# Lu-Zhan/Pano-NeRF

Hardware: AMD Instinct MI355X
Metric: rays/sec (train step) (higher is better)
Workload: dtype f32 (2xfp16 split products, fp32 accumulate; weight-gradient operands h_l / delta_l / r_l / hdot_l stored with 16 significant bits, 'Q24')

## Files before the change

pano-nerf_amd/csrc/pn_wgrad.hip:

```cpp
#include "pn_chain.h"

#ifdef PN_TRACE_WG
__device__ unsigned long long g_chain_trace[64];
extern "C" int pn_chain_trace_read(unsigned long long* out) {
    return hipMemcpyFromSymbol(out, HIP_SYMBOL(g_chain_trace), sizeof(unsigned long long) * 64) == hipSuccess ? 0 : -4;
}
#endif

struct WSeg {
    const float* X;
    const float* Y;
    int64_t nhalf;
    int FX, FY;
    int bias;
    const uint32_t* ax;
    const uint32_t* ay;
};
struct WgArgs {
    WSeg seg[4];
    int nseg;
    int64_t half_total, per;
    float* slab;
    int64_t slab_stride;
    int bias;
};
constexpr int WG_MAXJ = 8;
struct WgMulti {
    WgArgs job[WG_MAXJ];
};

template <int NP>
__device__ __forceinline__ f32x16 mfma_split32(const BFrag<NP>& a, const BFrag<NP>& b, f32x16 v) {
    if constexpr (NP == 3) {
        v = __builtin_amdgcn_mfma_f32_32x32x16_bf16(a.p[2], b.p[0], v, 0, 0, 0);
        v = __builtin_amdgcn_mfma_f32_32x32x16_bf16(a.p[0], b.p[2], v, 0, 0, 0);
        v = __builtin_amdgcn_mfma_f32_32x32x16_bf16(a.p[1], b.p[1], v, 0, 0, 0);
        v = __builtin_amdgcn_mfma_f32_32x32x16_bf16(a.p[1], b.p[0], v, 0, 0, 0);
        v = __builtin_amdgcn_mfma_f32_32x32x16_bf16(a.p[0], b.p[1], v, 0, 0, 0);
        v = __builtin_amdgcn_mfma_f32_32x32x16_bf16(a.p[0], b.p[0], v, 0, 0, 0);
    } else if constexpr (NP == 2) {
        v = __builtin_amdgcn_mfma_f32_32x32x16_f16(a.p[1], b.p[0], v, 0, 0, 0);
        v = __builtin_amdgcn_mfma_f32_32x32x16_f16(a.p[0], b.p[1], v, 0, 0, 0);
        v = __builtin_amdgcn_mfma_f32_32x32x16_f16(a.p[0], b.p[0], v, 0, 0, 0);
    } else {
        v = __builtin_amdgcn_mfma_f32_32x32x16_bf16(a.p[0], b.p[0], v, 0, 0, 0);
    }
    return v;
}
#define WG_LD(p) __builtin_nontemporal_load(p)
template <int NP, int TM, int TN, int WM, int WN, bool X24 = false, bool Y24 = false>
__global__ __launch_bounds__(64 * WM * WN) void k_chain_wgrad(WgMulti multi) {
    const WgArgs& a = multi.job[blockIdx.y];
    static_assert(!(X24 || Y24) || NP == 2, "Q24 tensors exist with fp16 pairs only");
    static_assert(!X24 || Y24, "combinations in use: (0,0), (0,1), (1,1)");
    constexpr bool ROT = X24 || Y24;
    constexpr int NTH = 64 * WM * WN, TMW = 32 * TM * WM, TNW = 32 * TN * WN;
    constexpr int PX = TMW * 16, PY = TNW * 16;
    constexpr int BUF = NP * (PX + PY);
    typedef typename TEl<NP>::type TE;
    constexpr int PPR = 16 * (int)sizeof(TE) / 16;
    constexpr int SPP = 16 / PPR;
    constexpr int CX = X24 ? 0 : TMW * PPR, CY = Y24 ? 0 : TNW * PPR;
    constexpr int LX = X24 ? 1 : (CX + NTH - 1) / NTH, LY = Y24 ? 1 : (CY + NTH - 1) / NTH;
    constexpr int UX = X24 ? TMW : 0, UY = Y24 ? TNW : 0;
    constexpr int LU = (UX + UY + NTH - 1) / NTH;
    static_assert(UX % 64 == 0, "a wave's units are all X or all Y");
    __shared__ __attribute__((aligned(16))) unsigned short smem[2 * BUF];
    const int tid = threadIdx.x, lane = tid & 63;
    const int wid = __builtin_amdgcn_readfirstlane(tid >> 6);
    const int wm = wid / WN, wn = wid % WN;
    const int64_t h0 = (int64_t)blockIdx.x * a.per;
    if (h0 >= a.half_total) return;
    int64_t h1 = h0 + a.per;
    if (h1 > a.half_total) h1 = a.half_total;

    f32x16 acc[TM][TN];
#pragma unroll
    for (int i = 0; i < TM; ++i)
#pragma unroll
        for (int j = 0; j < TN; ++j)
#pragma unroll
            for (int e = 0; e < 16; ++e) acc[i][j][e] = 0.f;
    float bsum[LX];
#pragma unroll
    for (int i = 0; i < LX; ++i) bsum[i] = 0.f;
    float bsum4[LU > 0 ? LU : 1][4] = {};

    constexpr int NSET = (X24 && LU == 1) ? 4 : ((NP <= 2 && (X24 ? 0 : LX) + (Y24 ? 0 : LY) + 3 * LU <= 4) ? 3 : 2);
    f32x4 xr[NSET][LX], yr[NSET][LY];
    f32x4 ur[NSET][LU > 0 ? LU : 1][3];
    constexpr bool ALT = (WM * WN == 8 && TM == 2 && TN == 4) && (X24 || Y24 || NP == 1);
    auto unit_of = [&](int i) { return tid + NTH * i; };
    float bw[NSET] = {};
    int sx[NSET] = {}, sy[NSET] = {}, unit = 0;
    auto seg_exps = [&](const WSeg& S, int& ex, int& ey) {
        ex = scale_exp(__uint_as_float(*S.ax), EXP_CAP_Z);
        ey = scale_exp(__uint_as_float(*S.ay), EXP_CAP_Z);
        int over = ex + ey - unit;
        const int rx = over < ex + 126 ? over : ex + 126;
        ex -= rx;
        ey -= over - rx;
        if (ey < -126) ey = -126;
    };
    if constexpr (NP == 2) {
        unit = 1 << 20;
        for (int i = 0; i < a.nseg; ++i) {
            const int e = scale_exp(__uint_as_float(*a.seg[i].ax), EXP_CAP_Z) + scale_exp(__uint_as_float(*a.seg[i].ay), EXP_CAP_Z);
            unit = e < unit ? e : unit;
        }
    }
    int csg = 0, cFX = a.seg[0].FX, cFY = a.seg[0].FY, csx = 0, csy = 0;
    int64_t cbase = 0, cend = a.seg[0].nhalf;
    const TE* cX = reinterpret_cast<const TE*>(a.seg[0].X);
    const TE* cY = reinterpret_cast<const TE*>(a.seg[0].Y);
    float cbw = a.seg[0].bias ? 1.f : 0.f;
    if constexpr (NP == 2) seg_exps(a.seg[0], csx, csy);
    auto load = [&](int64_t h, int set) __attribute__((always_inline)) {
        while (csg + 1 < a.nseg && h >= cend) {
            ++csg;
            const WSeg& S = a.seg[csg];
            cbase = cend;
            cend += S.nhalf;
            cX = reinterpret_cast<const TE*>(S.X);
            cY = reinterpret_cast<const TE*>(S.Y);
            cFX = S.FX;
            cFY = S.FY;
            cbw = S.bias ? 1.f : 0.f;
            if constexpr (NP == 2) seg_exps(S, csx, csy);
        }
        const int64_t hb = h - cbase;
        bw[set] = cbw;
        if constexpr (NP == 2) {
            sx[set] = csx;
            sy[set] = csy;
        }
        const int64_t blk = hb;
        const TE* xb = cX + blk * ((int64_t)cFX * TILE);
        const TE* yb = cY + blk * ((int64_t)cFY * TILE);
        if constexpr (!X24) {
#pragma unroll
            for (int i = 0; i < LX; ++i) {
                const int idx = tid + NTH * i;
                if (CX % NTH == 0 || idx < CX) xr[set][i] = WG_LD(reinterpret_cast<const f32x4*>(xb + (idx / PPR) * TILE + (idx % PPR) * SPP));
            }
        }
        if constexpr (!Y24) {
#pragma unroll
            for (int i = 0; i < LY; ++i) {
                const int idx = tid + NTH * i;
                if (CY % NTH == 0 || idx < CY) yr[set][i] = WG_LD(reinterpret_cast<const f32x4*>(yb + (idx / PPR) * TILE + (idx % PPR) * SPP));
            }
        }
        if constexpr (X24 || Y24) {
            const unsigned char* xq = reinterpret_cast<const unsigned char*>(cX) + blk * ((int64_t)cFX * 48);
            const unsigned char* yq = reinterpret_cast<const unsigned char*>(cY) + blk * ((int64_t)cFY * 48);
#pragma unroll
            for (int i = 0; i < LU; ++i) {
                const int u = unit_of(i);
                if ((UX + UY) % NTH == 0 || u < UX + UY) {
                    const f32x4* p = reinterpret_cast<const f32x4*>(u < UX ? xq + u * 48 : yq + (u - UX) * 48);
                    ur[set][i][0] = p[0];
                    ur[set][i][1] = p[1];
                    ur[set][i][2] = p[2];
                }
            }
        }
    };
    auto put = [&](unsigned short* plane0, int pstride, int idx, const f32x4& v, int ex) {
        if constexpr (NP == 1) {
            const int f = idx >> 1, q = idx & 1;
            *reinterpret_cast<f32x4*>(plane0 + f * 16 + ((q ^ ((f >> 3) & 1)) << 3)) = v;
            return;
        }
        const int f0 = idx >> 2, q = idx & 3;
        const int f = ROT ? ((f0 & ~3) | ((f0 + (f0 >> 2)) & 3)) : f0;
        const int o = f * 16 + (((q >> 1) ^ ((f >> 3) & 1)) << 3) + (q & 1) * 4;
        if constexpr (NP == 2) {
            const float s = pow2f(ex);
            const float x4[4] = {v[0], v[1], v[2], v[3]};
            uint32_t h2[2], l2[2];
            split2_pairs<2>(x4, s, h2, l2);
            *reinterpret_cast<uint2*>(plane0 + o) = make_uint2(h2[0], h2[1]);
            *reinterpret_cast<uint2*>(plane0 + pstride + o) = make_uint2(l2[0], l2[1]);
        } else {
            typedef __bf16 bf16x4 __attribute__((ext_vector_type(4)));
            bf16x4 hv, mv, lv;
#pragma unroll
            for (int c = 0; c < 4; ++c) {
                const __bf16 hb = (__bf16)v[c];
                hv[c] = hb;
                if constexpr (NP == 3) {
                    const float r1 = v[c] - (float)hb;
                    const __bf16 mb = (__bf16)r1;
                    mv[c] = mb;
                    lv[c] = (__bf16)(r1 - (float)mb);
                }
            }
            *reinterpret_cast<bf16x4*>(plane0 + o) = hv;
            if constexpr (NP == 3) {
                *reinterpret_cast<bf16x4*>(plane0 + pstride + o) = mv;
                *reinterpret_cast<bf16x4*>(plane0 + 2 * pstride + o) = lv;
            }
        }
    };
    auto put_unit = [&](unsigned short* plane0, int pstride, int u, const f32x4 (&r)[3], int ex, float* bs, float w) {
        typedef uint32_t u32x4 __attribute__((ext_vector_type(4)));
        uint32_t d[12];
#pragma unroll
        for (int k = 0; k < 3; ++k) {
            const u32x4 t = __builtin_bit_cast(u32x4, r[k]);
#pragma unroll
            for (int c = 0; c < 4; ++c) d[4 * k + c] = t[c];
        }
        float e[4][4];
#pragma unroll
        for (int sm = 0; sm < 4; ++sm) {
            e[sm][0] = __uint_as_float(d[3 * sm] << 8);
            e[sm][1] = __uint_as_float(__builtin_amdgcn_perm(d[3 * sm + 1], d[3 * sm], 0x0504030cu));
            e[sm][2] = __uint_as_float(__builtin_amdgcn_perm(d[3 * sm + 2], d[3 * sm + 1], 0x0403020cu));
            e[sm][3] = __uint_as_float(d[3 * sm + 2] & 0xffffff00u);
        }
        const int qb = u >> 2, sg = u & 3;
#pragma unroll
        for (int f = 0; f < 4; ++f) {
            const f32x4 v{e[0][f], e[1][f], e[2][f], e[3][f]};
            put(plane0, pstride, (4 * qb + f) * 4 + sg, v, ex);
            if (bs) bs[f] += w * ((v[0] + v[1]) + (v[2] + v[3]));
        }
    };
    auto stage = [&](int buf, int set) __attribute__((always_inline)) {
        unsigned short* xs = smem + buf * BUF;
        unsigned short* ys = xs + NP * PX;
        if constexpr (PN_ABL_WG & 2) {
            if constexpr (X24 || Y24) {
#pragma unroll
                for (int i = 0; i < LU; ++i) asm volatile("" ::"v"(ur[set][i][0]), "v"(ur[set][i][1]), "v"(ur[set][i][2]));
            }
            if constexpr (!X24) {
#pragma unroll
                for (int i = 0; i < LX; ++i) asm volatile("" ::"v"(xr[set][i]));
            }
            if constexpr (!Y24) {
#pragma unroll
                for (int i = 0; i < LY; ++i) asm volatile("" ::"v"(yr[set][i]));
            }
            return;
        }
        if constexpr (X24 || Y24) {
#pragma unroll
            for (int i = 0; i < LU; ++i) {
                const int u = unit_of(i);
                if ((UX + UY) % NTH == 0 || u < UX + UY) {
                    if (u < UX) put_unit(xs, PX, u, ur[set][i], sx[set], bsum4[i], bw[set]);
                    else put_unit(ys, PY, u - UX, ur[set][i], sy[set], nullptr, 0.f);
                }
            }
        }
        if constexpr (!X24)
#pragma unroll
        for (int i = 0; i < LX; ++i) {
            const int idx = tid + NTH * i;
            if (CX % NTH == 0 || idx < CX) {
                put(xs, PX, idx, xr[set][i], sx[set]);
                if constexpr (NP == 1) {
                    const bf16x8 hv = __builtin_bit_cast(bf16x8, xr[set][i]);
                    float t = 0.f;
#pragma unroll
                    for (int c = 0; c < 8; ++c) t += (float)hv[c];
                    bsum[i] += bw[set] * t;
                } else {
                    bsum[i] += bw[set] * ((xr[set][i][0] + xr[set][i][1]) + (xr[set][i][2] + xr[set][i][3]));
                }
            }
        }
        if constexpr (!Y24)
#pragma unroll
        for (int i = 0; i < LY; ++i) {
            const int idx = tid + NTH * i;
            if (CY % NTH == 0 || idx < CY) put(ys, PY, idx, yr[set][i], sy[set]);
        }
    };
    const int fr = lane & 31, fh = lane >> 5;
    auto frag = [&](const unsigned short* plane, int feature) {
        if constexpr (ROT) feature = (feature & ~3) | ((feature + (feature >> 2)) & 3);
        return *reinterpret_cast<const typename PlaneOf<NP>::type*>(plane + feature * 16 + ((fh ^ ((feature >> 3) & 1)) << 3));
    };
    auto compute = [&](int buf) __attribute__((always_inline)) {
        if constexpr (PN_ABL_WG & 1) return;
        const unsigned short* xs = smem + buf * BUF;
        const unsigned short* ys = xs + NP * PX;
        if constexpr (X24) {
            BFrag<NP> af[TM];
#pragma unroll
            for (int i = 0; i < TM; ++i)
#pragma unroll
                for (int p = 0; p < NP; ++p) af[i].p[p] = frag(xs + p * PX, 32 * (wm * TM + i) + fr);
#pragma unroll
            for (int j = 0; j < TN; ++j) {
                BFrag<NP> bf;
#pragma unroll
                for (int p = 0; p < NP; ++p) bf.p[p] = frag(ys + p * PY, 32 * (wn * TN + j) + fr);
#pragma unroll
                for (int i = 0; i < TM; ++i) acc[i][j] = mfma_split32<NP>(af[i], bf, acc[i][j]);
            }
            return;
        }
        typedef typename PlaneOf<NP>::type Frag;
        auto lds_of = [](const unsigned short* q) { return (uint32_t)(uintptr_t)(lds_ptr_t)q; };
        auto fidx = [&](int feature) {
            if constexpr (ROT) feature = (feature & ~3) | ((feature + (feature >> 2)) & 3);
            return feature * 16 + ((fh ^ ((feature >> 3) & 1)) << 3);
        };
        const uint32_t xa = lds_of(xs) + 2 * fidx(32 * (wm * TM) + fr), ya = lds_of(ys) + 2 * fidx(32 * (wn * TN) + fr);
        auto rd = [](Frag& dst, uint32_t addr, auto off) {
            asm volatile("ds_read_b128 %0, %1 offset:%2" : "=v"(dst) : "v"(addr), "n"(decltype(off)::value) : "memory");
        };
        static_assert(2 * NP * PX + 1024 * TM < 65536 && 2 * NP * PY + 1024 * TN < 65536, "16-bit offset field of ds_read_b128");
        BFrag<NP> af[TM];
        BFrag<NP> bf[2];
        auto read_b = [&](auto jc, BFrag<NP>& f) {
            constexpr int J = decltype(jc)::value;
            static_for<NP>([&](auto pc) {
                constexpr int P = decltype(pc)::value;
                rd(f.p[P], ya, std::integral_constant<int, 1024 * J + 2 * P * PY>{});
            });
        };
        auto settle = [&](auto left, BFrag<NP>& f) {
            constexpr int L = decltype(left)::value;
#pragma unroll
            for (int p = 0; p < NP; ++p) {
                if (p == 0) asm volatile("s_waitcnt lgkmcnt(%1)" : "+v"(f.p[p]) : "n"(L) : "memory");
                else asm volatile("" : "+v"(f.p[p]));
            }
        };
        read_b(std::integral_constant<int, 0>{}, bf[0]);
        static_for<TM>([&](auto ic) {
            constexpr int I = decltype(ic)::value;
            static_for<NP>([&](auto pc) {
                constexpr int P = decltype(pc)::value;
                rd(af[I].p[P], xa, std::integral_constant<int, 1024 * I + 2 * P * PX>{});
            });
        });
        if constexpr (TN > 1) {
            read_b(std::integral_constant<int, 1>{}, bf[1]);
            settle(std::integral_constant<int, NP>{}, bf[0]);
        } else {
            settle(std::integral_constant<int, 0>{}, bf[0]);
        }
#pragma unroll
        for (int i = 0; i < TM; ++i)
#pragma unroll
            for (int p = 0; p < NP; ++p) asm volatile("" : "+v"(af[i].p[p]));
        static_for<TN>([&](auto jc) {
            constexpr int J = decltype(jc)::value;
#pragma unroll
            for (int i = 0; i < TM; ++i) acc[i][J] = mfma_split32<NP>(af[i], bf[J & 1], acc[i][J]);
            if constexpr (J + 2 < TN) {
                __builtin_amdgcn_sched_barrier(0);
                read_b(std::integral_constant<int, J + 2>{}, bf[J & 1]);
            }
            if constexpr (J + 1 < TN) {
                if constexpr (J + 2 < TN) settle(std::integral_constant<int, NP>{}, bf[(J + 1) & 1]);
                else settle(std::integral_constant<int, 0>{}, bf[(J + 1) & 1]);
            }
        });
    };
#ifdef PN_TRACE_WG
    unsigned long long tw[4] = {0, 0, 0, 0};
#define WGT(i, expr)                                                   \
    do {                                                               \
        const unsigned long long t0_ = __builtin_amdgcn_s_memtime();   \
        expr;                                                          \
        asm volatile("s_waitcnt lgkmcnt(0)" ::: "memory");             \
        tw[i] += __builtin_amdgcn_s_memtime() - t0_;                   \
    } while (0)
#else
#define WGT(i, expr) expr
#endif
    auto one = [&](auto kc, int64_t h) __attribute__((always_inline)) {
        constexpr int K = decltype(kc)::value;
        if (h + K < h1) {
            WGT(0, stage(K % 2, K % NSET));
            WGT(1, __syncthreads());
            WGT(2, if (h + K + NSET < h1) load(h + K + NSET, K % NSET));
            WGT(3, compute(K % 2));
        }
    };
    if constexpr (ALT) {
        const int t = wid >= (WM * WN) / 2 ? 1 : 0;
        const int64_t n = h1 - h0;
        auto clampd = [&](int64_t hb) { return h0 + (hb < n ? hb : n - 1); };
        if (n > 0) {
            load(h0, 0);
            stage(0, 0);
            load(clampd(1), 0);
            if (t && 1 < n) stage(1, 0);
#pragma unroll
            for (int sidx = 1; sidx < NSET; ++sidx) load(clampd(sidx + t), sidx);
            load(clampd(NSET + t), 0);
            __syncthreads();
            constexpr int TRIPA = NSET == 3 ? 6 : (NSET == 4 ? 4 : 2);
            auto alt = [&](auto kc, auto guard, int64_t k0) __attribute__((always_inline)) {
                constexpr int K = decltype(kc)::value;
                if (!decltype(guard)::value || k0 + K < n) {
                    WGT(3, compute(K % 2));
                    if (t && !(PN_ABL_WG & 4)) WGT(1, __syncthreads());
                    const int64_t hb = k0 + K + 1 + t;
                    if (hb < n) WGT(0, stage((K + 1 + t) & 1, (K + 1) % NSET));
                    WGT(2, load(clampd(hb + NSET), (K + 1) % NSET));
                    if (!t && !(PN_ABL_WG & 4)) WGT(1, __syncthreads());
                }
            };
            int64_t k0 = 0;
            for (; k0 + TRIPA <= n; k0 += TRIPA) {
                alt(std::integral_constant<int, 0>{}, std::false_type{}, k0);
                alt(std::integral_constant<int, 1>{}, std::false_type{}, k0);
                if constexpr (TRIPA >= 4) {
                    alt(std::integral_constant<int, 2>{}, std::false_type{}, k0);
                    alt(std::integral_constant<int, 3>{}, std::false_type{}, k0);
                }
                if constexpr (TRIPA == 6) {
                    alt(std::integral_constant<int, 4>{}, std::false_type{}, k0);
                    alt(std::integral_constant<int, 5>{}, std::false_type{}, k0);
                }
            }
            if (k0 < n) {
                alt(std::integral_constant<int, 0>{}, std::true_type{}, k0);
                alt(std::integral_constant<int, 1>{}, std::true_type{}, k0);
                if constexpr (TRIPA >= 4) {
                    alt(std::integral_constant<int, 2>{}, std::true_type{}, k0);
                    alt(std::integral_constant<int, 3>{}, std::true_type{}, k0);
                }
                if constexpr (TRIPA == 6) {
                    alt(std::integral_constant<int, 4>{}, std::true_type{}, k0);
                    alt(std::integral_constant<int, 5>{}, std::true_type{}, k0);
                }
            }
        }
    } else
    if (h0 < h1) {
#pragma unroll
        for (int k = 0; k < NSET; ++k)
            if (h0 + k < h1) load(h0 + k, k);
        constexpr int TRIP = NSET == 3 ? 6 : (NSET == 4 ? 4 : 2);
        for (int64_t h = h0; h < h1; h += TRIP) {
            one(std::integral_constant<int, 0>{}, h);
            one(std::integral_constant<int, 1>{}, h);
            if constexpr (TRIP == 4) {
                one(std::integral_constant<int, 2>{}, h);
                one(std::integral_constant<int, 3>{}, h);
            }
            if constexpr (TRIP == 6) {
                one(std::integral_constant<int, 2>{}, h);
                one(std::integral_constant<int, 3>{}, h);
                one(std::integral_constant<int, 4>{}, h);
                one(std::integral_constant<int, 5>{}, h);
            }
        }
    }
#ifdef PN_TRACE_WG
    if (blockIdx.x == 0 && lane == 0 && (X24 && Y24)) {
#pragma unroll
        for (int i = 0; i < 4; ++i) g_chain_trace[8 * i + wid] = tw[i];
        if (wid == 0) g_chain_trace[32] = (unsigned long long)(h1 - h0);
    }
#endif
    float* out = a.slab + (int64_t)blockIdx.x * a.slab_stride;
#pragma unroll
    for (int i = 0; i < TM; ++i)
#pragma unroll
        for (int j = 0; j < TN; ++j)
#pragma unroll
            for (int e = 0; e < 16; ++e) {
                const int row = 32 * (wm * TM + i) + (e & 3) + 8 * (e >> 2) + 4 * fh;
                const float x = acc[i][j][e];
                out[(int64_t)row * TNW + 32 * (wn * TN + j) + fr] = NP == 2 ? ldexpf(x, -unit) : x;
            }
    if constexpr (X24) {
        if (a.bias) {
#pragma unroll
            for (int i = 0; i < LU; ++i) {
                const int u = tid + NTH * i;
#pragma unroll
                for (int f = 0; f < 4; ++f) {
                    float v = bsum4[i][f];
                    v += __shfl_xor(v, 1, 64);
                    v += __shfl_xor(v, 2, 64);
                    if ((u & 3) == 0 && u < UX) out[(int64_t)TMW * TNW + 4 * (u >> 2) + f] = v;
                }
            }
        }
    } else if (a.bias) {
#pragma unroll
        for (int i = 0; i < LX; ++i) {
            float v = bsum[i];
            v += __shfl_xor(v, 1, 64);
            if constexpr (PPR == 4) v += __shfl_xor(v, 2, 64);
            const int idx = tid + NTH * i;
            if (idx % PPR == 0 && (CX % NTH == 0 || idx < CX)) out[(int64_t)TMW * TNW + idx / PPR] = v;
        }
    }
}

struct WgJob {
    WSeg seg[4];
    int nseg;
    int cfg;
    int rows, cols;
    float* dst; int ldd;
    float* dbias;
    int fmt;
};
static const int kCfgM[5] = {256, 256, 128, 32, 32};
static const int kCfgN[5] = {256, 96, 288, 256, 128};

struct RedJob {
    const float* slabs;
    int64_t nb, stride, bias_off;
    int rows, cols, src_ld, ldd;
    float* dst;
    float* dbias;
};
constexpr int RED_MAXJ = WG_MAXJ;
struct RedMulti {
    RedJob job[RED_MAXJ];
};
__global__ __launch_bounds__(256) void k_reduce_job(RedMulti multi) {
    const RedJob& J = multi.job[blockIdx.y];
    const float* slabs = J.slabs;
    const int64_t nb = J.nb, stride = J.stride;
    const int rows = J.rows, cols = J.cols;
    float* dbias = J.dbias;
    __shared__ float red[4][64];
    const int tx = threadIdx.x & 63, ty = threadIdx.x >> 6;
    const int e = blockIdx.x * 64 + tx, nw = rows * cols, n = nw + (dbias ? rows : 0);
    if (blockIdx.x * 64 >= n) return;
    float acc = 0.f;
    float* d = nullptr;
    if (e < n) {
        const float* p;
        if (e < nw) {
            const int r = e / cols, c = e - r * cols;
            p = slabs + (int64_t)r * J.src_ld + c;
            d = J.dst + (int64_t)r * J.ldd + c;
        } else {
            p = slabs + J.bias_off + (e - nw);
            d = dbias + (e - nw);
        }
        int64_t b = ty;
        float a0 = 0.f, a1 = 0.f, a2 = 0.f, a3 = 0.f, a4 = 0.f, a5 = 0.f, a6 = 0.f, a7 = 0.f;
        for (; b + 28 < nb; b += 32) {
            a0 += p[b * stride];
            a1 += p[(b + 4) * stride];
            a2 += p[(b + 8) * stride];
            a3 += p[(b + 12) * stride];
            a4 += p[(b + 16) * stride];
            a5 += p[(b + 20) * stride];
            a6 += p[(b + 24) * stride];
            a7 += p[(b + 28) * stride];
        }
        for (; b < nb; b += 4) a0 += p[b * stride];
        acc = ((a0 + a1) + (a2 + a3)) + ((a4 + a5) + (a6 + a7));
    }
    red[ty][tx] = acc;
    __syncthreads();
    if (ty == 0 && e < n) *d += (red[0][tx] + red[1][tx]) + (red[2][tx] + red[3][tx]);
}

static int run_reduce(const std::vector<RedJob>& red, size_t i0, size_t i1, hipStream_t s);
template <int NP>
static int run_wgrad_group(const WgJob* jobs, int nj, float* work, int64_t work_floats, int max_wgs, hipStream_t s) {
    int64_t used = 0;
    std::vector<RedJob> red;
    if (nj < 1 || nj > WG_MAXJ) return PN_ERR_BAD_SHAPE;
    const WgJob& j0 = jobs[0];
    const int TMW = kCfgM[j0.cfg], TNW = kCfgN[j0.cfg];
    const int64_t stride = (int64_t)TMW * TNW + TMW;
    static const int kPerCu[5] = {1, 1, 1, 3, 4};
    int cus = chain_cus();
    if (max_wgs > 0 && max_wgs < cus) cus = max_wgs;
    const int64_t slots = (int64_t)cus * kPerCu[j0.cfg] / nj;
    WgMulti m{};
    int64_t nsplit_max = 0, slab0 = 0;
    float* const base = work + used;
    double flops = 0;
    for (int q = 0; q < nj; ++q) {
        const WgJob& j = jobs[q];
        if (j.cfg != j0.cfg || j.fmt != j0.fmt) return PN_ERR_BAD_SHAPE;
        WgArgs& a = m.job[q];
        int64_t total = 0;
        for (int i = 0; i < j.nseg; ++i) {
            a.seg[i] = j.seg[i];
            total += j.seg[i].nhalf;
        }
        a.nseg = j.nseg;
        a.half_total = total;
        int64_t nsplit = slots < 1 ? 1 : slots;
        if (nsplit > (total + 3) / 4) nsplit = (total + 3) / 4;
        if (nsplit < 1) nsplit = 1;
        a.per = (total + nsplit - 1) / nsplit;
        nsplit = (total + a.per - 1) / a.per;
        a.slab = base + slab0 * stride;
        a.slab_stride = stride;
        a.bias = j.dbias != nullptr;
        red.push_back(RedJob{a.slab, nsplit, stride, (int64_t)TMW * TNW, j.rows, j.cols, TNW, j.ldd, j.dst, j.dbias});
        slab0 += nsplit;
        nsplit_max = nsplit > nsplit_max ? nsplit : nsplit_max;
        double rows = 0;
        for (int i = 0; i < j.nseg; ++i) rows += 16.0 * (double)j.seg[i].nhalf;
        flops += 2.0 * rows * j.rows * j.cols;
    }
    if (used + slab0 * stride > work_floats) return PN_ERR_BAD_SHAPE;
    used += slab0 * stride;
    const dim3 grid((unsigned)nsplit_max, (unsigned)nj);
    const WgJob& j = j0;
    const WgMulti& a = m;
    {
    PnProfScope prof((j.cfg == 0 && j.fmt) ? (j.fmt == 3 ? 12 : 11) : 6 + j.cfg, flops, s);
    switch (j.cfg) {
        case 0:
            if constexpr (kQ24<NP>) {
                if (j.fmt == 3) { hipLaunchKernelGGL((k_chain_wgrad<NP, 2, 4, 4, 2, true, true>), grid, dim3(512), 0, s, a); break; }
                if (j.fmt == 1) { hipLaunchKernelGGL((k_chain_wgrad<NP, 2, 4, 4, 2, false, true>), grid, dim3(512), 0, s, a); break; }
            }
            if (j.fmt != 0) return PN_ERR_UNSUPPORTED;
            hipLaunchKernelGGL((k_chain_wgrad<NP, 2, 4, 4, 2>), grid, dim3(512), 0, s, a);
            break;
        case 1: hipLaunchKernelGGL((k_chain_wgrad<NP, 1, 3, 8, 1>), grid, dim3(512), 0, s, a); break;
        case 2: hipLaunchKernelGGL((k_chain_wgrad<NP, 1, 3, 4, 3>), grid, dim3(768), 0, s, a); break;
        case 3: hipLaunchKernelGGL((k_chain_wgrad<NP, 1, 2, 1, 4>), grid, dim3(256), 0, s, a); break;
        default: hipLaunchKernelGGL((k_chain_wgrad<NP, 1, 1, 1, 4>), grid, dim3(256), 0, s, a); break;
    }
    }
    PN_CHECK_LAUNCH();
    return run_reduce(red, 0, red.size(), s);
}
static int run_reduce(const std::vector<RedJob>& red, size_t i0, size_t i1, hipStream_t s) {
    while (i0 < i1) {
        const size_t n = i1 - i0 < (size_t)RED_MAXJ ? i1 - i0 : (size_t)RED_MAXJ;
        RedMulti r{};
        int nmax = 0;
        for (size_t q = 0; q < n; ++q) {
            r.job[q] = red[i0 + q];
            const int e = r.job[q].rows * r.job[q].cols + (r.job[q].dbias ? r.job[q].rows : 0);
            nmax = e > nmax ? e : nmax;
        }
        hipLaunchKernelGGL(k_reduce_job, dim3((unsigned)((nmax + 63) / 64), (unsigned)n), dim3(256), 0, s, r);
        PN_CHECK_LAUNCH();
        i0 += n;
    }
    return PN_OK;
}

extern "C" {

int64_t pn_chain_wgrad_work_floats(void) {
    const int64_t stride = 256 * 288 + 256;
    return (256 + 64) * stride + 1024;
}

int pn_chain_wgrad(int n, const PnChainEval* ev, int nc, int planes, float* grads, float* work, int64_t work_floats,
                   int which, int t_format, int max_wgs, void* stream) {
    if (n < 1 || n > 3 || which < 1 || which > 3 || max_wgs < 0) return PN_ERR_BAD_SHAPE;
    if (!tfmt_ok(planes, t_format)) return PN_ERR_UNSUPPORTED;
    const bool first = which & 1, second = which & 2;
    if (nc != 1 && nc != 5) return PN_ERR_UNSUPPORTED;
    if (planes != 1 && planes != 2 && planes != 3) return PN_ERR_UNSUPPORTED;
    if (!ev || !grads || !work) return PN_ERR_NULL;
    hipStream_t s = (hipStream_t)stream;
    const PnLayout L = pn_layout(nc);
    int n2 = 0;
    for (int e = 0; e < n; ++e) {
        if (ev[e].M <= 0 || !ev[e].enc_t || !ev[e].acts_t) return PN_ERR_NULL;
        if (first && (!ev[e].drgb_t || !ev[e].dhv_t || !ev[e].d8_t || !ev[e].delta_t)) return PN_ERR_NULL;
        if (ev[e].rs_t) {
            if (!ev[e].edot_t || !ev[e].tang_t || (first && !ev[e].coef_t)) return PN_ERR_NULL;
            if (second) ++n2;
        }
        if (planes == 2 && !ev[e].amax) return PN_ERR_NULL;
    }
    if ((first ? n : 0) + n2 > 4) return PN_ERR_UNSUPPORTED;
    if (!first && !n2) return PN_OK;
    std::vector<WgJob> jobs;
    std::vector<int> after;
    auto run = [&](const WgJob& j, int later = 0) {
        if (j.nseg) {
            jobs.push_back(j);
            after.push_back(later);
        }
        return (int)PN_OK;
    };
    auto am = [&](int e, int slot) -> const uint32_t* { return ev[e].amax ? ev[e].amax + slot : nullptr; };
    auto mp = [&](int e) { return pn_pad(ev[e].M); };
    const int64_t esz = planes == 1 ? 2 : 4;
    auto at = [&](const float* p, int64_t elems) { return reinterpret_cast<const float*>(reinterpret_cast<const char*>(p) + elems * esz); };
    auto act = [&](int e, int slot) { return at(ev[e].acts_t, act_off(slot, mp(e))); };
    int rc;
    for (int l = 0; l < 8; ++l) {
        WgJob j{};
        for (int e = 0; e < n; ++e) {
            const int64_t Mp = mp(e);
            if (first)
                j.seg[j.nseg++] = WSeg{at(ev[e].delta_t, (int64_t)l * Mp * 256), l == 0 ? ev[e].enc_t : act(e, l - 1), Mp / 16, 256,
                                       l == 0 ? 96 : 256, 1, am(e, AM_DELTA0 + l), am(e, l == 0 ? AM_ENC : AM_ACT0 + l - 1)};
            if (second && ev[e].rs_t)
                j.seg[j.nseg++] = WSeg{at(ev[e].rs_t, (int64_t)l * Mp * 256),
                                       l == 0 ? ev[e].edot_t : at(ev[e].tang_t, (int64_t)(l - 1) * Mp * 256), Mp / 16, 256,
                                       l == 0 ? 96 : 256, 0, am(e, AM_RS0 + l), am(e, l == 0 ? AM_EDOT : AM_TANG0 + l - 1)};
        }
        j.cfg = l == 0 ? 1 : 0;
        j.fmt = (t_format == 1 && l >= 1) ? (q24_delta(l) ? 3 : 1) : 0;
        j.rows = 256;
        j.cols = l == 0 ? 96 : 256;
        j.dst = grads + L.w[l];
        j.ldd = l == 0 ? 96 : (l == 5 ? 352 : 256);
        j.dbias = first ? grads + L.b[l] : nullptr;
        if ((rc = run(j)) != PN_OK) return rc;
        if (l == 5) {
            WgJob k{};
            for (int e = 0; e < n; ++e) {
                const int64_t Mp = mp(e);
                if (first)
                    k.seg[k.nseg++] = WSeg{at(ev[e].delta_t, (int64_t)5 * Mp * 256), ev[e].enc_t, Mp / 16, 256, 96, 0,
                                           am(e, AM_DELTA0 + 5), am(e, AM_ENC)};
                if (second && ev[e].rs_t)
                    k.seg[k.nseg++] = WSeg{at(ev[e].rs_t, (int64_t)5 * Mp * 256), ev[e].edot_t, Mp / 16, 256, 96, 0,
                                           am(e, AM_RS0 + 5), am(e, AM_EDOT)};
            }
            k.cfg = 1; k.rows = 256; k.cols = 96;
            k.dst = grads + L.w[5] + 256; k.ldd = 352; k.dbias = nullptr;
            if ((rc = run(k)) != PN_OK) return rc;
        }
    }
    if (first) {
        WgJob j{};
        for (int e = 0; e < n; ++e) j.seg[j.nseg++] = WSeg{ev[e].d8_t, act(e, 7), mp(e) / 16, 288, 256, 1, am(e, AM_D8B), am(e, AM_ACT0 + 7)};
        j.cfg = 0; j.rows = 256; j.cols = 256; j.dst = grads + L.we; j.ldd = 256; j.dbias = grads + L.be;
        if ((rc = run(j)) != PN_OK) return rc;
    }
    {
        WgJob j{};
        if (first)
            for (int e = 0; e < n; ++e) j.seg[j.nseg++] = WSeg{at(ev[e].d8_t, 256 * TILE), act(e, 7), mp(e) / 16, 288, 256, 1, am(e, AM_D8D), am(e, AM_ACT0 + 7)};
        j.cfg = 3; j.rows = nc; j.cols = 256; j.dst = grads + L.wd; j.ldd = 256; j.dbias = grads + L.bd;
        if ((rc = run(j)) != PN_OK) return rc;
        WgJob k{};
        for (int e = 0; e < n; ++e)
            if (first && ev[e].rs_t)
                k.seg[k.nseg++] = WSeg{ev[e].coef_t, at(ev[e].tang_t, (int64_t)7 * mp(e) * 256), mp(e) / 16, 32, 256, 0,
                                       am(e, AM_COEF), am(e, AM_TANG0 + 7)};
        if (k.nseg) {
            k.cfg = 3; k.rows = 1; k.cols = 256; k.dst = grads + L.wd; k.ldd = 256; k.dbias = nullptr;
            if ((rc = run(k, 1)) != PN_OK) return rc;
        }
    }
    if (first) {
        WgJob j{};
        for (int e = 0; e < n; ++e) j.seg[j.nseg++] = WSeg{ev[e].dhv_t, act(e, 8), mp(e) / 16, 128, 288, 1, am(e, AM_DHV), am(e, AM_ACT0 + 8)};
        j.cfg = 2; j.rows = 128; j.cols = PN_WIDTH + PN_VIEW_DIM; j.dst = grads + L.wv; j.ldd = PN_WIDTH + PN_VIEW_DIM;
        j.dbias = grads + L.bv;
        if ((rc = run(j)) != PN_OK) return rc;
    }
    if (first) {
        WgJob j{};
        for (int e = 0; e < n; ++e) j.seg[j.nseg++] = WSeg{ev[e].drgb_t, act(e, 9), mp(e) / 16, 32, 128, 1, am(e, AM_DRGB), am(e, AM_ACT0 + 9)};
        j.cfg = 4; j.rows = 3; j.cols = 128; j.dst = grads + L.wc; j.ldd = 128; j.dbias = grads + L.bc;
        if ((rc = run(j)) != PN_OK) return rc;
    }
    constexpr int64_t WG_RANGE = 512;
    std::vector<char> done(jobs.size(), 0);
    for (int pass = 0; pass < 2; ++pass)
    for (size_t i = 0; i < jobs.size(); ++i) {
        if (done[i] || after[i] != pass) continue;
        WgJob grp[WG_MAXJ];
        int ng = 0;
        int64_t total_i = 0;
        for (int q = 0; q < jobs[i].nseg; ++q) total_i += jobs[i].seg[q].nhalf;
        int cus_i = chain_cus();
        if (max_wgs > 0 && max_wgs < cus_i) cus_i = max_wgs;
        int64_t gmax = WG_RANGE * cus_i / (total_i > 0 ? total_i : 1);
        gmax = gmax < 1 ? 1 : (gmax > WG_MAXJ ? WG_MAXJ : gmax);
        for (size_t k = i; k < jobs.size() && ng < gmax; ++k)
            if (!done[k] && jobs[k].cfg == jobs[i].cfg && jobs[k].fmt == jobs[i].fmt && after[k] == after[i]) {
                grp[ng++] = jobs[k];
                done[k] = 1;
            }
        rc = planes == 3 ? run_wgrad_group<3>(grp, ng, work, work_floats, max_wgs, s)
                         : (planes == 2 ? run_wgrad_group<2>(grp, ng, work, work_floats, max_wgs, s)
                                        : run_wgrad_group<1>(grp, ng, work, work_floats, max_wgs, s));
        if (rc != PN_OK) return rc;
    }
    return PN_OK;
}

}
```

Measured before the change: 184,900.

## Stack layer-0 and layer-5 skip weight-gradient GEMMs sharing the encoding operand

Layer 0's weight gradient and the skip-connection part of layer 5's weight gradient both multiply a delta tensor by the same encoding input. This merges them into one stacked kernel configuration with 512 rows: half of each block's X tile comes from delta0 and half from delta5, and the Y (encoding) tile is loaded once and reused. Per-tensor scale exponents and a second reduction job handle the two outputs. The goal is to avoid reading the encoding twice and to drop one launch. In exchange the tile is larger, register pressure goes up, and the exponent handling gets more complicated.

```diff
diff --git a/pano-nerf_amd/csrc/pn_wgrad.hip b/pano-nerf_amd/csrc/pn_wgrad.hip
--- a/pano-nerf_amd/csrc/pn_wgrad.hip
+++ b/pano-nerf_amd/csrc/pn_wgrad.hip
@@ -15,6 +15,8 @@
     int bias;
     const uint32_t* ax;
     const uint32_t* ay;
+    const float* X2;
+    const uint32_t* ax2;
 };
 struct WgArgs {
     WSeg seg[4];
@@ -48,11 +50,12 @@
     return v;
 }
 #define WG_LD(p) __builtin_nontemporal_load(p)
-template <int NP, int TM, int TN, int WM, int WN, bool X24 = false, bool Y24 = false>
+template <int NP, int TM, int TN, int WM, int WN, bool X24 = false, bool Y24 = false, bool STK = false>
 __global__ __launch_bounds__(64 * WM * WN) void k_chain_wgrad(WgMulti multi) {
     const WgArgs& a = multi.job[blockIdx.y];
     static_assert(!(X24 || Y24) || NP == 2, "Q24 tensors exist with fp16 pairs only");
     static_assert(!X24 || Y24, "combinations in use: (0,0), (0,1), (1,1)");
+    static_assert(!STK || (!X24 && !Y24 && WN == 1 && WM % 2 == 0), "stacked X: fp32 / bf16 tensors, whole waves per row block");
     constexpr bool ROT = X24 || Y24;
     constexpr int NTH = 64 * WM * WN, TMW = 32 * TM * WM, TNW = 32 * TN * WN;
     constexpr int PX = TMW * 16, PY = TNW * 16;
@@ -65,6 +68,8 @@
     constexpr int UX = X24 ? TMW : 0, UY = Y24 ? TNW : 0;
     constexpr int LU = (UX + UY + NTH - 1) / NTH;
     static_assert(UX % 64 == 0, "a wave's units are all X or all Y");
+    static_assert(!STK || (CX % NTH == 0 && LX % 2 == 0), "stacked X: a thread's pieces split evenly between the two tensors");
+    constexpr int LXB = STK ? LX / 2 : LX;
     __shared__ __attribute__((aligned(16))) unsigned short smem[2 * BUF];
     const int tid = threadIdx.x, lane = tid & 63;
     const int wid = __builtin_amdgcn_readfirstlane(tid >> 6);
@@ -93,6 +98,7 @@
     auto unit_of = [&](int i) { return tid + NTH * i; };
     float bw[NSET] = {};
     int sx[NSET] = {}, sy[NSET] = {}, unit = 0;
+    int sx2[NSET] = {}, unit2 = 0;
     auto seg_exps = [&](const WSeg& S, int& ex, int& ey) {
         ex = scale_exp(__uint_as_float(*S.ax), EXP_CAP_Z);
         ey = scale_exp(__uint_as_float(*S.ay), EXP_CAP_Z);
@@ -102,19 +108,37 @@
         ey -= over - rx;
         if (ey < -126) ey = -126;
     };
+    auto seg_exps_stk = [&](const WSeg& S, int& ex, int& ex2, int& ey) {
+        ey = scale_exp(__uint_as_float(*S.ay), EXP_CAP_Z);
+        const int lo = (unit < unit2 ? unit : unit2) - ey;
+        int d = lo < -126 ? -126 - lo : 0;
+        d = d < ey + 126 ? d : ey + 126;
+        ey -= d;
+        ex = unit - ey;
+        ex2 = unit2 - ey;
+    };
     if constexpr (NP == 2) {
-        unit = 1 << 20;
+        unit = unit2 = 1 << 20;
         for (int i = 0; i < a.nseg; ++i) {
-            const int e = scale_exp(__uint_as_float(*a.seg[i].ax), EXP_CAP_Z) + scale_exp(__uint_as_float(*a.seg[i].ay), EXP_CAP_Z);
+            const int ey = scale_exp(__uint_as_float(*a.seg[i].ay), EXP_CAP_Z);
+            const int e = scale_exp(__uint_as_float(*a.seg[i].ax), EXP_CAP_Z) + ey;
             unit = e < unit ? e : unit;
-        }
-    }
-    int csg = 0, cFX = a.seg[0].FX, cFY = a.seg[0].FY, csx = 0, csy = 0;
+            if constexpr (STK) {
+                const int e2 = scale_exp(__uint_as_float(*a.seg[i].ax2), EXP_CAP_Z) + ey;
+                unit2 = e2 < unit2 ? e2 : unit2;
+            }
+        }
+    }
+    int csg = 0, cFX = a.seg[0].FX, cFY = a.seg[0].FY, csx = 0, csy = 0, csx2 = 0;
     int64_t cbase = 0, cend = a.seg[0].nhalf;
     const TE* cX = reinterpret_cast<const TE*>(a.seg[0].X);
     const TE* cY = reinterpret_cast<const TE*>(a.seg[0].Y);
+    const TE* cX2 = reinterpret_cast<const TE*>(a.seg[0].X2);
     float cbw = a.seg[0].bias ? 1.f : 0.f;
-    if constexpr (NP == 2) seg_exps(a.seg[0], csx, csy);
+    if constexpr (NP == 2) {
+        if constexpr (STK) seg_exps_stk(a.seg[0], csx, csx2, csy);
+        else seg_exps(a.seg[0], csx, csy);
+    }
     auto load = [&](int64_t h, int set) __attribute__((always_inline)) {
         while (csg + 1 < a.nseg && h >= cend) {
             ++csg;
@@ -123,21 +147,33 @@
             cend += S.nhalf;
             cX = reinterpret_cast<const TE*>(S.X);
             cY = reinterpret_cast<const TE*>(S.Y);
+            cX2 = reinterpret_cast<const TE*>(S.X2);
             cFX = S.FX;
             cFY = S.FY;
             cbw = S.bias ? 1.f : 0.f;
-            if constexpr (NP == 2) seg_exps(S, csx, csy);
+            if constexpr (NP == 2) {
+                if constexpr (STK) seg_exps_stk(S, csx, csx2, csy);
+                else seg_exps(S, csx, csy);
+            }
         }
         const int64_t hb = h - cbase;
         bw[set] = cbw;
         if constexpr (NP == 2) {
             sx[set] = csx;
             sy[set] = csy;
+            if constexpr (STK) sx2[set] = csx2;
         }
         const int64_t blk = hb;
         const TE* xb = cX + blk * ((int64_t)cFX * TILE);
         const TE* yb = cY + blk * ((int64_t)cFY * TILE);
-        if constexpr (!X24) {
+        if constexpr (STK) {
+            const TE* xb2 = cX2 + blk * ((int64_t)cFX * TILE);
+#pragma unroll
+            for (int i = 0; i < LX; ++i) {
+                const int idx = tid + NTH * i - (i < LX / 2 ? 0 : CX / 2);
+                xr[set][i] = WG_LD(reinterpret_cast<const f32x4*>((i < LX / 2 ? xb : xb2) + (idx / PPR) * TILE + (idx % PPR) * SPP));
+            }
+        } else if constexpr (!X24) {
 #pragma unroll
             for (int i = 0; i < LX; ++i) {
                 const int idx = tid + NTH * i;
@@ -176,7 +212,7 @@
         const int f = ROT ? ((f0 & ~3) | ((f0 + (f0 >> 2)) & 3)) : f0;
         const int o = f * 16 + (((q >> 1) ^ ((f >> 3) & 1)) << 3) + (q & 1) * 4;
         if constexpr (NP == 2) {
-            const float s = pow2f(ex);
+            const float s = (STK && (ex < -126 || ex > 127)) ? 0.f : pow2f(ex);
             const float x4[4] = {v[0], v[1], v[2], v[3]};
             uint32_t h2[2], l2[2];
             split2_pairs<2>(x4, s, h2, l2);
@@ -261,7 +297,8 @@
         for (int i = 0; i < LX; ++i) {
             const int idx = tid + NTH * i;
             if (CX % NTH == 0 || idx < CX) {
-                put(xs, PX, idx, xr[set][i], sx[set]);
+                put(xs, PX, idx, xr[set][i], (STK && i >= LX / 2) ? sx2[set] : sx[set]);
+                if (i >= LXB) continue;
                 if constexpr (NP == 1) {
                     const bf16x8 hv = __builtin_bit_cast(bf16x8, xr[set][i]);
                     float t = 0.f;
@@ -474,7 +511,7 @@
             for (int e = 0; e < 16; ++e) {
                 const int row = 32 * (wm * TM + i) + (e & 3) + 8 * (e >> 2) + 4 * fh;
                 const float x = acc[i][j][e];
-                out[(int64_t)row * TNW + 32 * (wn * TN + j) + fr] = NP == 2 ? ldexpf(x, -unit) : x;
+                out[(int64_t)row * TNW + 32 * (wn * TN + j) + fr] = NP == 2 ? ldexpf(x, -((STK && wm >= WM / 2) ? unit2 : unit)) : x;
             }
     if constexpr (X24) {
         if (a.bias) {
@@ -492,7 +529,7 @@
         }
     } else if (a.bias) {
 #pragma unroll
-        for (int i = 0; i < LX; ++i) {
+        for (int i = 0; i < LXB; ++i) {
             float v = bsum[i];
             v += __shfl_xor(v, 1, 64);
             if constexpr (PPR == 4) v += __shfl_xor(v, 2, 64);
@@ -509,10 +546,12 @@
     int rows, cols;
     float* dst; int ldd;
     float* dbias;
+    float* dst2; int ldd2;
     int fmt;
 };
-static const int kCfgM[5] = {256, 256, 128, 32, 32};
-static const int kCfgN[5] = {256, 96, 288, 256, 128};
+static const int kCfgM[6] = {256, 256, 128, 32, 32, 512};
+static const int kCfgN[6] = {256, 96, 288, 256, 128, 96};
+static constexpr bool kStacked[4] = {false, true, true, true};
 
 struct RedJob {
     const float* slabs;
@@ -576,7 +615,7 @@
     const WgJob& j0 = jobs[0];
     const int TMW = kCfgM[j0.cfg], TNW = kCfgN[j0.cfg];
     const int64_t stride = (int64_t)TMW * TNW + TMW;
-    static const int kPerCu[5] = {1, 1, 1, 3, 4};
+    static const int kPerCu[6] = {1, 1, 1, 3, 4, 1};
     int cus = chain_cus();
     if (max_wgs > 0 && max_wgs < cus) cus = max_wgs;
     const int64_t slots = (int64_t)cus * kPerCu[j0.cfg] / nj;
@@ -604,11 +643,13 @@
         a.slab_stride = stride;
         a.bias = j.dbias != nullptr;
         red.push_back(RedJob{a.slab, nsplit, stride, (int64_t)TMW * TNW, j.rows, j.cols, TNW, j.ldd, j.dst, j.dbias});
+        if (j.cfg == 5)
+            red.push_back(RedJob{a.slab + (int64_t)(TMW / 2) * TNW, nsplit, stride, 0, j.rows, j.cols, TNW, j.ldd2, j.dst2, nullptr});
         slab0 += nsplit;
         nsplit_max = nsplit > nsplit_max ? nsplit : nsplit_max;
         double rows = 0;
         for (int i = 0; i < j.nseg; ++i) rows += 16.0 * (double)j.seg[i].nhalf;
-        flops += 2.0 * rows * j.rows * j.cols;
+        flops += 2.0 * rows * j.rows * j.cols * (j.cfg == 5 ? 2 : 1);
     }
     if (used + slab0 * stride > work_floats) return PN_ERR_BAD_SHAPE;
     used += slab0 * stride;
@@ -616,7 +657,7 @@
     const WgJob& j = j0;
     const WgMulti& a = m;
     {
-    PnProfScope prof((j.cfg == 0 && j.fmt) ? (j.fmt == 3 ? 12 : 11) : 6 + j.cfg, flops, s);
+    PnProfScope prof((j.cfg == 0 && j.fmt) ? (j.fmt == 3 ? 12 : 11) : (j.cfg == 5 ? 7 : 6 + j.cfg), flops, s);
     switch (j.cfg) {
         case 0:
             if constexpr (kQ24<NP>) {
@@ -629,6 +670,10 @@
         case 1: hipLaunchKernelGGL((k_chain_wgrad<NP, 1, 3, 8, 1>), grid, dim3(512), 0, s, a); break;
         case 2: hipLaunchKernelGGL((k_chain_wgrad<NP, 1, 3, 4, 3>), grid, dim3(768), 0, s, a); break;
         case 3: hipLaunchKernelGGL((k_chain_wgrad<NP, 1, 2, 1, 4>), grid, dim3(256), 0, s, a); break;
+        case 5:
+            if constexpr (kStacked[NP]) hipLaunchKernelGGL((k_chain_wgrad<NP, 2, 3, 8, 1, false, false, true>), grid, dim3(512), 0, s, a);
+            else return PN_ERR_UNSUPPORTED;
+            break;
         default: hipLaunchKernelGGL((k_chain_wgrad<NP, 1, 1, 1, 4>), grid, dim3(256), 0, s, a); break;
     }
     }
@@ -696,17 +741,21 @@
     auto at = [&](const float* p, int64_t elems) { return reinterpret_cast<const float*>(reinterpret_cast<const char*>(p) + elems * esz); };
     auto act = [&](int e, int slot) { return at(ev[e].acts_t, act_off(slot, mp(e))); };
     int rc;
+    const bool stacked = kStacked[planes];
     for (int l = 0; l < 8; ++l) {
         WgJob j{};
+        const bool stk = stacked && l == 0;
         for (int e = 0; e < n; ++e) {
             const int64_t Mp = mp(e);
             if (first)
                 j.seg[j.nseg++] = WSeg{at(ev[e].delta_t, (int64_t)l * Mp * 256), l == 0 ? ev[e].enc_t : act(e, l - 1), Mp / 16, 256,
-                                       l == 0 ? 96 : 256, 1, am(e, AM_DELTA0 + l), am(e, l == 0 ? AM_ENC : AM_ACT0 + l - 1)};
+                                       l == 0 ? 96 : 256, 1, am(e, AM_DELTA0 + l), am(e, l == 0 ? AM_ENC : AM_ACT0 + l - 1),
+                                       stk ? at(ev[e].delta_t, (int64_t)5 * Mp * 256) : nullptr, stk ? am(e, AM_DELTA0 + 5) : nullptr};
             if (second && ev[e].rs_t)
                 j.seg[j.nseg++] = WSeg{at(ev[e].rs_t, (int64_t)l * Mp * 256),
                                        l == 0 ? ev[e].edot_t : at(ev[e].tang_t, (int64_t)(l - 1) * Mp * 256), Mp / 16, 256,
-                                       l == 0 ? 96 : 256, 0, am(e, AM_RS0 + l), am(e, l == 0 ? AM_EDOT : AM_TANG0 + l - 1)};
+                                       l == 0 ? 96 : 256, 0, am(e, AM_RS0 + l), am(e, l == 0 ? AM_EDOT : AM_TANG0 + l - 1),
+                                       stk ? at(ev[e].rs_t, (int64_t)5 * Mp * 256) : nullptr, stk ? am(e, AM_RS0 + 5) : nullptr};
         }
         j.cfg = l == 0 ? 1 : 0;
         j.fmt = (t_format == 1 && l >= 1) ? (q24_delta(l) ? 3 : 1) : 0;
@@ -715,8 +764,13 @@
         j.dst = grads + L.w[l];
         j.ldd = l == 0 ? 96 : (l == 5 ? 352 : 256);
         j.dbias = first ? grads + L.b[l] : nullptr;
+        if (stk) {
+            j.cfg = 5;
+            j.dst2 = grads + L.w[5] + 256;
+            j.ldd2 = 352;
+        }
         if ((rc = run(j)) != PN_OK) return rc;
-        if (l == 5) {
+        if (l == 5 && !stacked) {
             WgJob k{};
             for (int e = 0; e < n; ++e) {
                 const int64_t Mp = mp(e);
```

Result: no change. 186,200 (median of 6 runs) (+0.7%).
